# heitorrapela/HalluciDet

Hardware: AMD Instinct MI355X
Metric: images/sec train_hallucidet (640x512, batch 8/GPU) (higher is better)
Workload: dtype f16; 1 GPU; train_hallucidet.py fasterrcnn LLVIP batch=8 fp16 on 1xMI355X (BASELINE configs[1]); U-Net resnet34 fwd+bwd, 3 frozen Faster R-CNN R50-FPN passes @300x300 (one batched evaluation of 24 images: trunk, RPN, RoI heads, NMS for all three; the RGB / IR passes' LOSS VALUES, which the reference computes and discards, are not evaluated), loss scaling, value clip 0.5, Adam; global_batch=8, image=1x512x640 IR + 3x512x640 RGB, batch_per_gpu=8, parallelism=dp1

## Files before the change

### hallucidet_amd/csrc/gemm_w8.hip

```cpp
#include "hd_common.h"
#include "conv_params.h"
#include "hd_lds_dma.h"

namespace {

constexpr int GK = 64;
constexpr int GROW = 64;

template <int BM, int BN, int NSTAGE>
__global__ __launch_bounds__(128 * (BM / 64)) void gemm_w8_kernel(ConvP p) {
  static_assert((BM == 256 || BM == 128) && BN == 128, "tile");
  constexpr int NWM = BM / 64, NT = 128 * NWM, RP = NT / 8;
  constexpr int NA = BN / 64;
  constexpr int NB = 2;
  constexpr int STAGE = (BM + BN) * GROW;
  constexpr int W_PASS = BN / RP, X_PASS = BM / RP;
  constexpr int L_TILE = W_PASS + X_PASS;
  static_assert(NSTAGE * STAGE * 2 <= 160 * 1024, "LDS");
  static_assert(W_PASS >= 1 && X_PASS >= 1, "a DMA pass covers RP rows");
  __shared__ __attribute__((aligned(1024))) f16 lds[NSTAGE * STAGE];

  const int tid = threadIdx.x, lane = tid & 63;
  const int wave = __builtin_amdgcn_readfirstlane(tid >> 6);
  const int wn = wave / NWM, wm = wave - wn * NWM;

  const int bid = hd_xcd_contiguous(blockIdx.x, gridDim.x);
  int tile_m, tile_n;
  hd_conv_tile_of(p, bid, tile_m, tile_n);
  const int m0 = tile_m * BM, n0 = tile_n * BN;
  const int K = p.Ktot;

  const __amdgpu_buffer_rsrc_t rx = __builtin_amdgcn_make_buffer_rsrc(const_cast<f16*>(p.x), 0, p.xbytes, 0x00020000);
  const __amdgpu_buffer_rsrc_t rw = __builtin_amdgcn_make_buffer_rsrc(const_cast<f16*>(p.w), 0, p.wbytes, 0x00020000);

  const int j = (tid & 7) ^ ((tid >> 4) & 7);
  unsigned wbase[W_PASS], xbase[X_PASS];
  bool wok[W_PASS], xok[X_PASS];
#pragma unroll
  for (int i = 0; i < W_PASS; ++i) {
    const int row = n0 + i * RP + (tid >> 3);
    wok[i] = row < p.Cout;
    wbase[i] = (unsigned)(wok[i] ? row : 0) * (unsigned)K * 2u + (unsigned)j * 16u;
  }
#pragma unroll
  for (int i = 0; i < X_PASS; ++i) {
    const int row = m0 + i * RP + (tid >> 3);
    xok[i] = row < p.M;
    xbase[i] = (unsigned)(xok[i] ? row : 0) * (unsigned)K * 2u + (unsigned)j * 16u;
  }
  const int nk = (K + GK - 1) / GK;
  int kt_issue = 0;
  auto gload = [&](int stage) {
    f16* sw = lds + stage * STAGE + wave * (8 * GROW);
    f16* sx = sw + BN * GROW;
    const bool kv = kt_issue * GK + j * 8 < K;
    const unsigned ko = (unsigned)kt_issue * (GK * 2);
#pragma unroll
    for (int i = 0; i < W_PASS; ++i) dma16(rw, sw + i * (RP * GROW), (wok[i] && kv) ? wbase[i] + ko : OOB);
#pragma unroll
    for (int i = 0; i < X_PASS; ++i) dma16(rx, sx + i * (RP * GROW), (xok[i] && kv) ? xbase[i] + ko : OOB);
    ++kt_issue;
  };

  f32x16 acc[NA][NB];
#pragma unroll
  for (int a = 0; a < NA; ++a)
#pragma unroll
    for (int b = 0; b < NB; ++b)
#pragma unroll
      for (int r = 0; r < 16; ++r) acc[a][b][r] = 0.f;

  const int frow = lane & 31, fh = lane >> 5, swz = (frow >> 1) & 7;
  f16x8 wf[2][NA], xf[2][NB];
  auto frag = [&](int stage, int ks, int buf) {
    const f16* sw = lds + stage * STAGE;
    const f16* sx = sw + BN * GROW;
    const int slot = ((ks * 2 + fh) ^ swz) * 8;
#pragma unroll
    for (int a = 0; a < NA; ++a) wf[buf][a] = *reinterpret_cast<const f16x8*>(sw + (wn * (BN / 2) + a * 32 + frow) * GROW + slot);
#pragma unroll
    for (int b = 0; b < NB; ++b) xf[buf][b] = *reinterpret_cast<const f16x8*>(sx + (wm * 64 + b * 32 + frow) * GROW + slot);
  };

#pragma unroll
  for (int t = 0; t < NSTAGE - 1; ++t) gload(t);
  int rd = 0, wr = NSTAGE - 1;
  for (int kt = 0; kt < nk; ++kt) {
    asm volatile("s_waitcnt vmcnt(%0)" ::"n"((NSTAGE - 2) * L_TILE) : "memory");
    __builtin_amdgcn_s_barrier();
    __builtin_amdgcn_sched_barrier(0);
    frag(rd, 0, 0);
    frag(rd, 1, 1);
    __builtin_amdgcn_sched_barrier(0);
    gload(wr);
#pragma unroll
    for (int ks = 0; ks < GK / 16; ++ks) {
      __builtin_amdgcn_sched_barrier(0);
#pragma unroll
      for (int a = 0; a < NA; ++a)
#pragma unroll
        for (int b = 0; b < NB; ++b) acc[a][b] = __builtin_amdgcn_mfma_f32_32x32x16_f16(wf[ks & 1][a], xf[ks & 1][b], acc[a][b], 0, 0, 0);
      __builtin_amdgcn_sched_barrier(0);
      if (ks + 2 < GK / 16) frag(rd, ks + 2, ks & 1);
    }
    rd = (rd + 1 == NSTAGE) ? 0 : rd + 1;
    wr = (wr + 1 == NSTAGE) ? 0 : wr + 1;
  }
  asm volatile("s_waitcnt vmcnt(0)" ::: "memory");

  f16* __restrict__ yp = reinterpret_cast<f16*>(p.y);
  const f16* __restrict__ maskp = p.mask;
  const f16* __restrict__ resp = p.res;
  const float* __restrict__ biasp = p.bias;
  const bool relu = p.act == HD_ACT_RELU;
  const int N = p.Cout;
#pragma unroll
  for (int a = 0; a < NA; ++a) {
    const int cb = n0 + wn * (BN / 2) + a * 32;
#pragma unroll
    for (int gp = 0; gp < 4; gp += 2) {
      f32x4 bv[2] = {{0.f, 0.f, 0.f, 0.f}, {0.f, 0.f, 0.f, 0.f}};
      if (biasp) {
#pragma unroll
        for (int gg = 0; gg < 2; ++gg) {
          const int c = cb + 8 * (gp + gg) + 4 * fh;
          if (c < N) bv[gg] = *reinterpret_cast<const f32x4*>(biasp + c);
        }
      }
      const int co = cb + 8 * (gp + fh);
#pragma unroll
      for (int b = 0; b < NB; ++b) {
        const int m = m0 + wm * 64 + b * 32 + frow;
        const bool ok = m < p.M && co < N;
        unsigned pk[2][2];
#pragma unroll
        for (int gg = 0; gg < 2; ++gg) {
          float v[4];
          f16x4 rv = {(f16)0.f, (f16)0.f, (f16)0.f, (f16)0.f};
          if (resp) {
            const int c = cb + 8 * (gp + gg) + 4 * fh;
            if (m < p.M && c < N) rv = *reinterpret_cast<const f16x4*>(resp + (size_t)m * N + c);
          }
#pragma unroll
          for (int i = 0; i < 4; ++i) {
            v[i] = acc[a][b][4 * (gp + gg) + i];
            if (resp) v[i] += (float)rv[i];
            v[i] += bv[gg][i];
            if (relu) v[i] = fmaxf(v[i], 0.f);
          }
          const f16x2 o01 = {(f16)v[0], (f16)v[1]}, o23 = {(f16)v[2], (f16)v[3]};
          pk[gg][0] = __builtin_bit_cast(unsigned, o01);
          pk[gg][1] = __builtin_bit_cast(unsigned, o23);
        }
        const auto q0 = __builtin_amdgcn_permlane32_swap(pk[0][0], pk[1][0], false, false);
        const auto q1 = __builtin_amdgcn_permlane32_swap(pk[0][1], pk[1][1], false, false);
        u32x4 o = {q0[0], q1[0], q0[1], q1[1]};
        if (ok) {
          const size_t off = (size_t)m * N + co;
          if (maskp) {
            const f16x8 mv = *reinterpret_cast<const f16x8*>(maskp + off);
            f16x8 ov = __builtin_bit_cast(f16x8, o);
#pragma unroll
            for (int k = 0; k < 8; ++k) ov[k] = ((float)mv[k] > 0.f) ? ov[k] : (f16)0.f;
            o = __builtin_bit_cast(u32x4, ov);
          }
          *reinterpret_cast<u32x4*>(yp + off) = o;
        }
      }
    }
  }
}

}

bool hd_gemm_w8_eligible(const ConvP& p) {
  const bool flat = (p.KH == 1 && p.KW == 1 && p.stride == 1 && p.pad == 0) ||
                    (p.KH == p.Hsrc && p.KW == p.Wsrc && p.pad == 0 && p.Ho == 1 && p.Wo == 1);
  return flat && !p.x2 && !p.up1 && p.in_dil == 1 && !p.stats && !p.in_scale && !p.bs_y && p.out_mode == HD_OUT_NHWC_F16 &&
         (p.act == HD_ACT_NONE || p.act == HD_ACT_RELU) && (p.Cout % 8) == 0 && (p.Ktot % 64) == 0 && (p.Hin == p.Hsrc && p.Win == p.Wsrc);
}

void hd_gemm_w8_launch(ConvP& p, int tile, hipStream_t s) {
  const int bm = tile == 1128 ? 128 : 256;
  p.gm = hd_cdiv(p.M, bm);
  p.gn = hd_cdiv(p.Cout, 128);
  p.tgroup = hd_conv_tile_order(p);
  if (tile == 128) hipLaunchKernelGGL((gemm_w8_kernel<256, 128, 3>), dim3(p.gm * p.gn), dim3(512), 0, s, p);
  else hipLaunchKernelGGL((gemm_w8_kernel<128, 128, 2>), dim3(p.gm * p.gn), dim3(256), 0, s, p);
}
```

Baseline: 831.7 images/s.

## Ping-pong two wave groups in 8-wave 1x1 GEMM and use 8 waves for small grids

Splits the 8-wave GEMM into two 4-wave groups that alternate between LDS fragment load plus DMA issue and an MFMA phase at raised priority, coordinated by barriers, so memory and matrix work from different groups overlap. It also adds a 128x128 tile variant with 8 waves and 4 stages for launches whose tile count fits within the CU count, to lift per-CU occupancy on small grids. The cost is more registers for holding all K-step fragments, more barriers, and more LDS for the deeper pipeline.

```diff
diff --git a/hallucidet_amd/csrc/gemm_w8.hip b/hallucidet_amd/csrc/gemm_w8.hip
--- a/hallucidet_amd/csrc/gemm_w8.hip
+++ b/hallucidet_amd/csrc/gemm_w8.hip
@@ -7,12 +7,13 @@
 constexpr int GK = 64;
 constexpr int GROW = 64;
 
-template <int BM, int BN, int NSTAGE>
-__global__ __launch_bounds__(128 * (BM / 64)) void gemm_w8_kernel(ConvP p) {
-  static_assert((BM == 256 || BM == 128) && BN == 128, "tile");
-  constexpr int NWM = BM / 64, NT = 128 * NWM, RP = NT / 8;
+template <int BM, int BN, int NW, int NSTAGE>
+__global__ __launch_bounds__(64 * NW) void gemm_w8_kernel(ConvP p) {
+  static_assert((BM == 256 || BM == 128) && BN == 128 && (NW == 8 || NW == 4), "tile");
+  constexpr int NWM = NW / 2, NT = 64 * NW, RP = NT / 8;
   constexpr int NA = BN / 64;
-  constexpr int NB = 2;
+  constexpr int NB = BM / NWM / 32;
+  static_assert(NB == 1 || NB == 2, "wave tile");
   constexpr int STAGE = (BM + BN) * GROW;
   constexpr int W_PASS = BN / RP, X_PASS = BM / RP;
   constexpr int L_TILE = W_PASS + X_PASS;
@@ -71,7 +72,8 @@
       for (int r = 0; r < 16; ++r) acc[a][b][r] = 0.f;
 
   const int frow = lane & 31, fh = lane >> 5, swz = (frow >> 1) & 7;
-  f16x8 wf[2][NA], xf[2][NB];
+  constexpr int NFB = NW == 8 ? GK / 16 : 2;
+  f16x8 wf[NFB][NA], xf[NFB][NB];
   auto frag = [&](int stage, int ks, int buf) {
     const f16* sw = lds + stage * STAGE;
     const f16* sx = sw + BN * GROW;
@@ -79,32 +81,84 @@
 #pragma unroll
     for (int a = 0; a < NA; ++a) wf[buf][a] = *reinterpret_cast<const f16x8*>(sw + (wn * (BN / 2) + a * 32 + frow) * GROW + slot);
 #pragma unroll
-    for (int b = 0; b < NB; ++b) xf[buf][b] = *reinterpret_cast<const f16x8*>(sx + (wm * 64 + b * 32 + frow) * GROW + slot);
+    for (int b = 0; b < NB; ++b) xf[buf][b] = *reinterpret_cast<const f16x8*>(sx + (wm * (NB * 32) + b * 32 + frow) * GROW + slot);
   };
 
 #pragma unroll
   for (int t = 0; t < NSTAGE - 1; ++t) gload(t);
   int rd = 0, wr = NSTAGE - 1;
-  for (int kt = 0; kt < nk; ++kt) {
-    asm volatile("s_waitcnt vmcnt(%0)" ::"n"((NSTAGE - 2) * L_TILE) : "memory");
+  if constexpr (NW == 8) {
+    static_assert(NSTAGE >= 3, "a tile is waited for one K step after it was issued");
+    constexpr int N_FLY = (NSTAGE - 2) * L_TILE;
+    const int grp = __builtin_amdgcn_readfirstlane(wave >> 2);
+    auto load_phase = [&]() {
+      __builtin_amdgcn_sched_barrier(0);
+#pragma unroll
+      for (int ks = 0; ks < GK / 16; ++ks) frag(rd, ks, ks);
+      __builtin_amdgcn_sched_barrier(0);
+      gload(wr);
+      __builtin_amdgcn_sched_barrier(0);
+    };
+    auto mfma_phase = [&]() {
+      __builtin_amdgcn_sched_barrier(0);
+      __builtin_amdgcn_s_setprio(1);
+#pragma unroll
+      for (int ks = 0; ks < GK / 16; ++ks)
+#pragma unroll
+        for (int a = 0; a < NA; ++a)
+#pragma unroll
+          for (int b = 0; b < NB; ++b) acc[a][b] = __builtin_amdgcn_mfma_f32_32x32x16_f16(wf[ks][a], xf[ks][b], acc[a][b], 0, 0, 0);
+      __builtin_amdgcn_s_setprio(0);
+      __builtin_amdgcn_sched_barrier(0);
+    };
+    auto advance = [&]() {
+      rd = (rd + 1 == NSTAGE) ? 0 : rd + 1;
+      wr = (wr + 1 == NSTAGE) ? 0 : wr + 1;
+    };
+    asm volatile("s_waitcnt vmcnt(%0)" ::"n"(N_FLY) : "memory");
     __builtin_amdgcn_s_barrier();
-    __builtin_amdgcn_sched_barrier(0);
-    frag(rd, 0, 0);
-    frag(rd, 1, 1);
-    __builtin_amdgcn_sched_barrier(0);
-    gload(wr);
-#pragma unroll
-    for (int ks = 0; ks < GK / 16; ++ks) {
-      __builtin_amdgcn_sched_barrier(0);
-#pragma unroll
-      for (int a = 0; a < NA; ++a)
-#pragma unroll
-        for (int b = 0; b < NB; ++b) acc[a][b] = __builtin_amdgcn_mfma_f32_32x32x16_f16(wf[ks & 1][a], xf[ks & 1][b], acc[a][b], 0, 0, 0);
-      __builtin_amdgcn_sched_barrier(0);
-      if (ks + 2 < GK / 16) frag(rd, ks + 2, ks & 1);
+    if (grp == 0) {
+      for (int kt = 0; kt < nk; ++kt) {
+        load_phase();
+        asm volatile("s_waitcnt lgkmcnt(0)" ::: "memory");
+        __builtin_amdgcn_s_barrier();
+        mfma_phase();
+        asm volatile("s_waitcnt vmcnt(%0)" ::"n"(N_FLY) : "memory");
+        __builtin_amdgcn_s_barrier();
+        advance();
+      }
+    } else {
+      for (int kt = 0; kt < nk; ++kt) {
+        __builtin_amdgcn_s_barrier();
+        load_phase();
+        asm volatile("s_waitcnt vmcnt(%0) lgkmcnt(0)" ::"n"(N_FLY) : "memory");
+        __builtin_amdgcn_s_barrier();
+        mfma_phase();
+        advance();
+      }
     }
-    rd = (rd + 1 == NSTAGE) ? 0 : rd + 1;
-    wr = (wr + 1 == NSTAGE) ? 0 : wr + 1;
+  } else {
+    for (int kt = 0; kt < nk; ++kt) {
+      asm volatile("s_waitcnt vmcnt(%0)" ::"n"((NSTAGE - 2) * L_TILE) : "memory");
+      __builtin_amdgcn_s_barrier();
+      __builtin_amdgcn_sched_barrier(0);
+      frag(rd, 0, 0);
+      frag(rd, 1, 1);
+      __builtin_amdgcn_sched_barrier(0);
+      gload(wr);
+#pragma unroll
+      for (int ks = 0; ks < GK / 16; ++ks) {
+        __builtin_amdgcn_sched_barrier(0);
+#pragma unroll
+        for (int a = 0; a < NA; ++a)
+#pragma unroll
+          for (int b = 0; b < NB; ++b) acc[a][b] = __builtin_amdgcn_mfma_f32_32x32x16_f16(wf[ks & 1][a], xf[ks & 1][b], acc[a][b], 0, 0, 0);
+        __builtin_amdgcn_sched_barrier(0);
+        if (ks + 2 < GK / 16) frag(rd, ks + 2, ks & 1);
+      }
+      rd = (rd + 1 == NSTAGE) ? 0 : rd + 1;
+      wr = (wr + 1 == NSTAGE) ? 0 : wr + 1;
+    }
   }
   asm volatile("s_waitcnt vmcnt(0)" ::: "memory");
 
@@ -130,7 +184,7 @@
       const int co = cb + 8 * (gp + fh);
 #pragma unroll
       for (int b = 0; b < NB; ++b) {
-        const int m = m0 + wm * 64 + b * 32 + frow;
+        const int m = m0 + wm * (NB * 32) + b * 32 + frow;
         const bool ok = m < p.M && co < N;
         unsigned pk[2][2];
 #pragma unroll
@@ -181,10 +235,12 @@
 }
 
 void hd_gemm_w8_launch(ConvP& p, int tile, hipStream_t s) {
+  constexpr int CUS = 256;
   const int bm = tile == 1128 ? 128 : 256;
   p.gm = hd_cdiv(p.M, bm);
   p.gn = hd_cdiv(p.Cout, 128);
   p.tgroup = hd_conv_tile_order(p);
-  if (tile == 128) hipLaunchKernelGGL((gemm_w8_kernel<256, 128, 3>), dim3(p.gm * p.gn), dim3(512), 0, s, p);
-  else hipLaunchKernelGGL((gemm_w8_kernel<128, 128, 2>), dim3(p.gm * p.gn), dim3(256), 0, s, p);
-}
+  if (tile == 128) hipLaunchKernelGGL((gemm_w8_kernel<256, 128, 8, 3>), dim3(p.gm * p.gn), dim3(512), 0, s, p);
+  else if ((int64_t)p.gm * p.gn <= CUS) hipLaunchKernelGGL((gemm_w8_kernel<128, 128, 8, 4>), dim3(p.gm * p.gn), dim3(512), 0, s, p);
+  else hipLaunchKernelGGL((gemm_w8_kernel<128, 128, 4, 2>), dim3(p.gm * p.gn), dim3(256), 0, s, p);
+}
```

Measured after the change: 839.9 images/s (median of 6 runs). About the same (+1.0%).
